# louisaslett/PhaseType

Hardware: NVIDIA B200
Metric: path_draws_per_sec (higher is better)
Workload: dtype f64

## Files before the change

### phasetype_b200/csrc/k_mhrs.cu

```cuda
#include <cooperative_groups.h>
#include "engine_internal.h"
#include "pht_philox.h"

namespace cg = cooperative_groups;

#ifndef MHRS_THREADS
#define MHRS_THREADS 256
#endif
#define MHRS_WARPS (MHRS_THREADS / 32)
#ifndef MHRS_MIN_BLOCKS
#define MHRS_MIN_BLOCKS 4
#endif
#ifndef MHRS_TAIL_MIN_BLOCKS
#define MHRS_TAIL_MIN_BLOCKS 3
#endif
#ifndef MHRS_NOINLINE_COLD
#define MHRS_COLD static __device__ __forceinline__
#else
#define MHRS_COLD static __device__ __noinline__
#endif
#define GUIDE_BITS 8
#define GUIDE (1 << GUIDE_BITS)
#ifndef END_CAP
#define END_CAP 32u
#endif
#ifndef MHRS_REPLAY_MIN_BLOCKS
#define MHRS_REPLAY_MIN_BLOCKS 4
#endif
#ifndef REPLAY_REFILL_MIN
#define REPLAY_REFILL_MIN 16
#endif
#ifndef EV_MIN
#define EV_MIN 8u
#endif
#ifndef EV_WAIT
#define EV_WAIT 16u
#endif
#ifndef PREFETCH_MIN
#define PREFETCH_MIN 8
#endif
#ifndef TAIL_CH
#define TAIL_CH 256u
#endif
#ifndef TAIL_BATCH
#define TAIL_BATCH 1u
#endif
#ifndef TAIL_LATE_P
#define TAIL_LATE_P 1024u
#endif
#ifndef TAIL_LATE_GROWTH
#define TAIL_LATE_GROWTH 4u
#endif
#ifndef DRAIN_LANES
#define DRAIN_LANES 32
#endif
#ifndef TAIL_K0
#define TAIL_K0 512u
#endif
#define TAIL_KMAX (1u << 24)
#ifndef TAIL_GROWTH
#define TAIL_GROWTH 2u
#endif
#ifndef FOUND_PERIOD
#define FOUND_PERIOD 8u
#endif
#define POOL_MIN 32u
#ifndef POOL_MAX
#define POOL_MAX 256u
#endif
#define FOUND_NONE 0xFFFFFFFFFFFFFFFFull
#define T52_NEVER (1ull << 52)
#define LOWBITS (1u << 20)
#define XBAR_TIMEOUT_NS 4000000000ull

#define RF_PROP 2u
#define RF_OFF 4u
#define RF_SKIP 8u

template <int NC>
struct MhrsSmem {
    static constexpr int R = NC + 1;
    unsigned long long thr[R * R];
    double cum[R * R];
    double scale[NC];
    double s[NC];
    double inv_smax;
    unsigned long long zlo[NC];
    long long zhi[NC];
    unsigned int Nacc[NC * NC];
    unsigned int Bacc[NC];
    float A[R + 3];
    unsigned int paths_done;
    unsigned int scan[MHRS_WARPS + 1];
    uint32_t pctr[MHRS_WARPS];
    float pf_yf[MHRS_THREADS]; uint32_t pf_og[MHRS_THREADS], pf_pos[MHRS_THREADS];
    uint32_t mh_cur_a[MHRS_THREADS], mh_misc[MHRS_THREADS];
    unsigned char guide[R * GUIDE];
};

__device__ __forceinline__ unsigned long long gtimer() {
    unsigned long long t; asm volatile("mov.u64 %0, %globaltimer;" : "=l"(t)); return t;
}
__device__ __forceinline__ float lg2_approx(float x) {
    float r; asm("lg2.approx.ftz.f32 %0, %1;" : "=f"(r) : "f"(x)); return r;
}

__device__ __forceinline__ pht_u32x4 philox_block(uint32_t c0, uint32_t c1, uint32_t c2, uint32_t c3, const SweepParams &p) {
    PHT_PHILOX_ROUND(p.rk.k[0], p.rk.k[1])   PHT_PHILOX_ROUND(p.rk.k[2], p.rk.k[3])   PHT_PHILOX_ROUND(p.rk.k[4], p.rk.k[5])
    PHT_PHILOX_ROUND(p.rk.k[6], p.rk.k[7])   PHT_PHILOX_ROUND(p.rk.k[8], p.rk.k[9])   PHT_PHILOX_ROUND(p.rk.k[10], p.rk.k[11])
    PHT_PHILOX_ROUND(p.rk.k[12], p.rk.k[13]) PHT_PHILOX_ROUND(p.rk.k[14], p.rk.k[15]) PHT_PHILOX_ROUND(p.rk.k[16], p.rk.k[17])
    PHT_PHILOX_ROUND(p.rk.k[18], p.rk.k[19])
    pht_u32x4 out; out.v[0] = c0; out.v[1] = c1; out.v[2] = c2; out.v[3] = c3;
    return out;
}

struct Walk {
    double t, spare;
    uint32_t spare_hi, a, b;
    int j;
    bool odd, fresh;
};
struct Rec { double lastt; int B; long out_idx; double *z2; };

__device__ __forceinline__ void walk_begin(Walk &w, uint32_t a, bool off, uint32_t og, const SweepParams &p, uint32_t iter) {
    w.a = a; w.fresh = true; w.b = 0; w.odd = false; w.t = 0.0; w.j = 0; w.spare = 0.0; w.spare_hi = 0u;
    if (off) {
        pht_u32x4 r = philox_block(0u, a, og, iter, p);
        w.spare = pht_u01(r.v[2], r.v[3]); w.spare_hi = r.v[3]; w.odd = true; w.b = 1;
    }
}

__device__ __forceinline__ double log_unit(double x) { return pht_log_core(pht_d2u(x), 0); }

template <bool RECORD, int NC>
__device__ __forceinline__ bool walk_step(Walk &w, double y, bool cens, uint32_t og, const SweepParams &p, MhrsSmem<NC> &sm,
                                          uint32_t iter, int n, Rec &rec) {
    constexpr int R = NC + 1;
    pht_u32x4 r = philox_block(w.b, w.a, og, iter, p);
    w.b++;
    const double f = pht_u01(r.v[0], r.v[1]), g = pht_u01(r.v[2], r.v[3]);
    const double uA = w.odd ? w.spare : f;
    const uint32_t hiA = w.odd ? w.spare_hi : r.v[1];
    const double uB = w.odd ? f : g;
    w.spare = g; w.spare_hi = r.v[3];
    const bool fresh = w.fresh;
    const int row = fresh ? n : w.j;
    const int last = fresh ? n - 1 : n;
    const double *c = sm.cum + row * R;
    int k = sm.guide[row * GUIDE + (hiA >> (32 - GUIDE_BITS))] & 0x7f;
    while (k < last && c[k] < uA) k++;
    const bool cont = (k < n) && (w.t < y || cens);
    const bool ended = !fresh && !cont;
    const bool advance = !fresh && cont;
    if (RECORD) {
        if (advance) {
            rec.z2[w.j] += w.t - rec.lastt;
            if (p.outN != nullptr) p.outN[(size_t)rec.out_idx * n * n + w.j + k * n]++;
            else atomicAdd(&sm.Nacc[w.j + k * n], 1u);
        }
        rec.lastt = fresh ? 0.0 : (advance ? w.t : rec.lastt);
        rec.B = fresh ? k : rec.B;
    }
    const double tb = fresh ? 0.0 : w.t;
    const int jn = ended ? w.j : k;
    const double tn = tb + sm.scale[jn] * (-log_unit(uB));
    w.t = ended ? w.t : tn;
    w.j = jn;
    w.fresh = false;
    return ended;
}

template <int NC, bool IV = false>
MHRS_COLD uint32_t exact_attempt(uint32_t a, bool off, double y, bool cens, uint32_t og, const SweepParams &p,
                                                      MhrsSmem<NC> &sm, uint32_t iter, int n, uint32_t smask, double u = 0.0) {
    Walk w; Rec norec; norec.lastt = 0.0; norec.B = 0; norec.out_idx = 0; norec.z2 = nullptr;
    walk_begin(w, a, off, og, p, iter);
    unsigned st = 1;
    while (!walk_step<false>(w, y, cens, og, p, sm, iter, n, norec)) st++;
    bool ok = (w.t >= y) && ((smask >> w.j) & 1u);
    if constexpr (IV) ok = ok && w.t <= u;
    return (ok ? 1u : 0u) | ((uint32_t)w.j << 8) | ((st > 0xffffu ? 0xffffu : st) << 16);
}

template <int NC>
__device__ __forceinline__ void replay_phase(const SweepParams &p, MhrsSmem<NC> &sm, uint32_t iter, int n,
                                             uint32_t obs_begin, uint32_t obs_end, unsigned &c_jumps) {
    const unsigned FULL = 0xffffffffu; const int lane = threadIdx.x & 31;
    constexpr bool LANE_Z = NC <= 8;
    long long ztot[LANE_Z ? NC : 1];
#pragma unroll
    for (int i = 0; i < (LANE_Z ? NC : 1); i++) ztot[i] = 0;
    double z2[NC];
    Walk w; Rec rec; rec.lastt = 0.0; rec.B = 0; rec.z2 = z2; rec.out_idx = 0;
    w.t = 0.0; w.spare = 0.0; w.spare_hi = 0u; w.a = 0u; w.b = 0u; w.j = 0; w.odd = false; w.fresh = true;
    double y = 0.0; bool cens = false, act = false, fin = false, dry = false, bad = false; uint32_t og = 0u;
    unsigned paths = 0;
    const double zs = pht_u2d((uint64_t)(1023 + p.zbits) << 52);
    for (;;) {
        const unsigned idle = __ballot_sync(FULL, !act);
        if (idle == FULL || (unsigned)__popc(idle) >= REPLAY_REFILL_MIN) {
            if (fin) {
                fin = false; paths++;
                z2[w.j] += (cens ? w.t : y) - rec.lastt;
                if (p.outB != nullptr) {
                    p.outB[rec.out_idx] = rec.B;
                    p.outN[rec.out_idx * n * n + w.j + w.j * n]++;
#pragma unroll 1
                    for (int i = 0; i < n; i++) p.outz[rec.out_idx * n + i] = z2[i];
                } else {
                    atomicAdd(&sm.Nacc[w.j + w.j * n], 1u); atomicAdd(&sm.Bacc[rec.B], 1u);
#pragma unroll
                    for (int i = 0; i < NC; i++) {
                        if (i < n) {
                            const double v = z2[i];
                            bad = bad || !(v * zs < 4.0e18);
                            const long long fx = __double2ll_rn(v * zs);
                            if (LANE_Z) { ztot[LANE_Z ? i : 0] += fx; bad = bad || ztot[LANE_Z ? i : 0] < 0; }
                            else if (fx != 0) pht_zfix_add(sm.zlo, sm.zhi, i, fx);
                        }
                    }
                }
            }
            if (!dry) {
                const unsigned cnt = __popc(idle);
                unsigned long long base = 0;
                if (lane == 0) base = (unsigned long long)obs_begin + atomicAdd(&p.state->replay_next, (unsigned long long)cnt);
                base = __shfl_sync(FULL, base, 0);
                const unsigned long long left = base < obs_end ? (unsigned long long)obs_end - base : 0ull;
                const unsigned avail = left < cnt ? (unsigned)left : cnt;
                if (avail < cnt) dry = true;
                const unsigned rank = __popc(idle & ((1u << lane) - 1u));
                if (!act && rank < avail) {
                    const unsigned long long pos = base + rank;
                    const uint4 r = p.recs[pos];
                    if (!(r.z & RF_SKIP)) {
                        const uint32_t obs_local = p.perm ? p.perm[pos] : (uint32_t)pos;
                        y = p.y[pos]; cens = p.cens[pos] != 0; og = p.obs_rank + obs_local * p.obs_world;
                        rec.out_idx = (long)obs_local - p.first; rec.lastt = 0.0; rec.B = 0;
                        uint32_t a = r.x;
                        if (r.z & RF_PROP) {
                            const pht_u32x4 q = philox_block(0u, r.y + 1u, og, iter, p);
                            const double U = pht_u01(q.v[0], q.v[1]);
                            if (U < sm.s[(r.z >> 16) & 0xffu] / sm.s[(r.z >> 8) & 0xffu]) a = r.y;
                        }
#pragma unroll
                        for (int i = 0; i < NC; i++) z2[i] = 0.0;
                        walk_begin(w, a, (r.z & RF_OFF) != 0u, og, p, iter);
                        act = true;
                    }
                }
            }
        }
        if (__ballot_sync(FULL, act) == 0u) { if (dry) break; else continue; }
        __syncwarp();
        if (act) { c_jumps++; if (walk_step<true>(w, y, cens, og, p, sm, iter, n, rec)) { act = false; fin = true; } }
    }
    if (p.outB == nullptr) {
        if (LANE_Z) {
#pragma unroll
            for (int i = 0; i < NC; i++) {
                if (i < n) {
                    const long long fx = ztot[LANE_Z ? i : 0];
                    unsigned long long lo = (unsigned long long)fx & 0xffffffffull; long long hi = fx >> 32;
                    for (int d = 16; d > 0; d >>= 1) { lo += __shfl_xor_sync(FULL, lo, d); hi += __shfl_xor_sync(FULL, hi, d); }
                    if (lane == 0 && (lo | (unsigned long long)hi)) {
                        atomicAdd(&sm.zlo[i], lo); atomicAdd(reinterpret_cast<unsigned long long *>(&sm.zhi[i]), (unsigned long long)hi);
                    }
                }
            }
        }
        if (bad) atomicOr(&p.state->error, 2);
    }
    for (int d = 16; d > 0; d >>= 1) paths += __shfl_xor_sync(FULL, paths, d);
    if (lane == 0 && paths) atomicAdd(&sm.paths_done, paths);
}

struct ObsF { float yn; uint32_t og; bool cens; };
__device__ __forceinline__ void obs_set(ObsF &o, float yn, uint32_t og, bool cens) { o.yn = yn; o.og = og; o.cens = cens; }
struct ObsFU : ObsF { float un, bn; };
template <bool IV> struct ObsOf { typedef ObsF T; };
template <> struct ObsOf<true> { typedef ObsFU T; };
__device__ __forceinline__ void obs_set_u(ObsF &, float) {}
__device__ __forceinline__ void obs_set_u(ObsFU &o, float un) { o.un = un; o.bn = (un < __int_as_float(0x7f800000)) ? un : o.yn; }
__device__ __forceinline__ float obs_bound(const ObsF &o) { return o.yn; }
__device__ __forceinline__ float obs_bound(const ObsFU &o) { return o.bn; }
template <bool IV> __device__ __forceinline__ double upper_at(const double *u, uint32_t pos) {
    if constexpr (IV) return u[pos]; else return 0.0;
}
struct Fast { float t, dacc; uint32_t a, b; int row; };

__device__ __forceinline__ void fast_begin(Fast &f, uint32_t a, int n) { f.t = 0.0f; f.dacc = 0.0f; f.a = a; f.b = 0u; f.row = n; }

template <int NC, bool IV = false>
__device__ __forceinline__ void fast_step(Fast &f, const typename ObsOf<IV>::T &o, const SweepParams &p, const MhrsSmem<NC> &sm, uint32_t iter, int n,
                                          bool &fail, bool &surv, bool &amb, int &kout) {
    constexpr int R = NC + 1;
    const pht_u32x4 r = philox_block(f.b, f.a, o.og, iter, p);
    f.b++;
    const unsigned long long x = (((unsigned long long)r.v[1] << 32) | r.v[0]) >> 12;
    const unsigned g = sm.guide[f.row * GUIDE + (r.v[1] >> (32 - GUIDE_BITS))];
    int k = (int)(g & 0x7fu);
    if (!(g & 0x80u)) { const unsigned long long *th = sm.thr + f.row * R; while (x >= th[k]) k++; }
    const uint32_t w = r.v[3];
    const uint32_t wb = __float_as_uint(__uint2float_rn(w));
    const uint32_t eb = wb >> 23;
    const float lg2m = lg2_approx(__uint_as_float((wb & 0x007fffffu) | 0x3f800000u));
    const float L = (__uint_as_float(0x4b400000u + eb) - 12583071.0f) + lg2m;
    f.t = __fmaf_rn(L, sm.A[k], f.t);
    const float trunc = __uint_as_float((254u - eb) << 23);
    const float c0y = __fmaf_rn(1.2e-7f, obs_bound(o), 4.5e-7f);
    const float step_err = __fmaf_rn(trunc, 2.0f, __fmaf_rn(fabsf(L), 2.5e-7f, c0y));
    const bool flagged = (w < 4096u) || (f.b >> 12) != 0u;
    f.dacc = flagged ? __int_as_float(0x7f800000) : f.dacc + step_err;
    const bool absd = (k == n);
    const float diff = f.t - o.yn;
    const bool over = diff > f.dacc, under = -diff > f.dacc;
    const bool test = o.cens == absd;
    surv = test && over;
    amb = test && !over && !under;
    fail = absd && (!o.cens || under);
    if constexpr (IV) {
        const float du = f.t - o.un;
        const bool past = du > f.dacc, below = -du > f.dacc;
        fail = fail || past;
        amb = test && !under && !past && !(over && below);
        surv = surv && below;
    }
    kout = absd ? f.row : k;
    f.row = k;
}

template <int NC>
__device__ __forceinline__ void build_tables(const SweepParams &p, MhrsSmem<NC> &sm, int n, const ModelLayout &ML) {
    constexpr int R = NC + 1;
    const int tid = threadIdx.x;
    double smax = 0.0;
    for (int i = 0; i < n; i++) { const double sc = p.model[ML.scale + i]; smax = (sc > smax) ? sc : smax; }
    const double inv_smax = 1.0 / smax;
    for (int i = tid; i < n; i += MHRS_THREADS) {
        const double sc = p.model[ML.scale + i];
        sm.scale[i] = sc; sm.s[i] = p.model[ML.s + i]; sm.zlo[i] = 0ull; sm.zhi[i] = 0; sm.Bacc[i] = 0u;
        sm.A[i] = (float)((-0.69314718055994530942 * sc) * inv_smax);
    }
    if (tid == 0) { sm.A[n] = 0.0f; sm.inv_smax = inv_smax; }
    for (int i = tid; i < n * n; i += MHRS_THREADS) sm.Nacc[i] = 0u;
    for (int e = tid; e < R * R; e += MHRS_THREADS) {
        const int row = e / R, k = e % R;
        unsigned long long t52 = T52_NEVER; double c = 0.0;
        if (row <= n && k <= n) {
            c = p.model[ML.cum + row * (n + 1) + k];
            const int last = (row == n) ? n - 1 : n;
            if (k < last && c < 1.0) {
                if (!(c > 0.0)) t52 = 0ull;
                else {
                    const unsigned long long xf = (unsigned long long)(c * 4503599627370496.0);
                    const double u = pht_u2d(0x3ff0000000000000ULL | xf) - 0.99999999999999988898;
                    t52 = (u > c) ? xf : xf + 1ull;
                }
            }
        }
        sm.thr[e] = t52; sm.cum[e] = c;
    }
    if (tid == 0) sm.paths_done = 0u;
    __syncthreads();
    for (int e = tid; e < (n + 1) * GUIDE; e += MHRS_THREADS) {
        const int row = e / GUIDE, b = e % GUIDE, last = (row == n) ? n - 1 : n;
        const double floor_u = (double)b * (1.0 / GUIDE);
        int k = 0;
        while (k < last && sm.cum[row * R + k] <= floor_u) k++;
        const bool pure = sm.thr[row * R + k] >= ((unsigned long long)(b + 1) << (52 - GUIDE_BITS));
        sm.guide[e] = (unsigned char)(k | (pure ? 0x80 : 0));
    }
    __syncthreads();
}

__device__ __forceinline__ uint32_t pack_flags(bool have_cur, bool cur_off, bool off, bool cens, int cur_pre, uint32_t kprop) {
    return (have_cur ? TI_HAVE : 0u) | (cur_off ? TI_CUROFF : 0u) | (off ? TI_OFF : 0u) | (cens ? TI_CENS : 0u) |
           ((uint32_t)(cur_pre & 0xff) << 8) | (kprop << 16);
}

__device__ __forceinline__ void peer_barrier(cg::grid_group &grid, const SweepParams &p, unsigned long long epoch) {
    const unsigned long long t_in = (blockIdx.x == 0 && threadIdx.x == 0) ? gtimer() : 0ull;
    __threadfence_system();
    grid.sync();
    if (blockIdx.x == 0) {
        const int t = threadIdx.x;
        if (t < (int)p.obs_world && p.state->xdead == 0u) {
            volatile unsigned long long *mine = &p.xpeer[t]->flags[p.obs_rank];
            __threadfence_system();
            *mine = epoch;
            __threadfence_system();
            volatile unsigned long long *theirs = &p.xw->flags[t];
            const unsigned long long t0 = gtimer();
            while (*theirs < epoch) {
                if (gtimer() - t0 > XBAR_TIMEOUT_NS) { p.state->xdead = 1u; atomicOr(&p.state->error, 64); break; }
            }
            __threadfence_system();
        }
    }
    grid.sync();
    if (blockIdx.x == 0 && threadIdx.x == 0) atomicAdd(&p.state->counters[PHT_CNT_NS_XWAIT], gtimer() - t_in);
}

struct TailView {
    TailItem *items; const uint32_t *pend; unsigned long long *found; uint32_t P, K;
    bool global; uint32_t parity;
    const double *u;
};

template <int NC, bool IV = false>
__device__ __forceinline__ void tail_search(const TailView &tv, const SweepParams &p, MhrsSmem<NC> &sm, uint32_t iter, int n,
                                            uint32_t smask, uint32_t nwarps,
                                            unsigned &c_jumps, unsigned &c_attempts) {
    const unsigned FULL = 0xffffffffu; const int lane = threadIdx.x & 31;
    const uint32_t W = tv.global ? p.obs_world : 1u;
    const uint32_t Pl = (tv.P + W - 1u) / W;
    const unsigned long long total_units = (unsigned long long)Pl * tv.K;
    Fast f; fast_begin(f, 0u, n);
    typename ObsOf<IV>::T mo; obs_set(mo, 0.0f, 0u, false); obs_set_u(mo, 0.0f);
    uint32_t my_item = 0xFFFFFFFFu; bool active = false;
    unsigned steps = 0;
    uint32_t *ctr = &sm.pctr[threadIdx.x >> 5];
    if (lane == 0) *ctr = 0u;
    __syncwarp();
    unsigned long long u_next = 0, u_end = 0, last_base = 0, remaining = total_units;
    bool out_of_units = false, finished = false;
    uint32_t item = 0, og = 0, a_first = 0, pool_end = 0; float yf = 0.0f, uf = 0.0f; bool cens = false, first_off = false;
    while (!finished) {
        bool want_exact = false, exact_off = false, survived = false; int kend = 0;
#define TAIL_GRAB() do { \
            const uint32_t na_ = atomicAdd(ctr, 1u); \
            if (na_ < pool_end) { \
                my_item = item; obs_set(mo, yf, og, cens); obs_set_u(mo, uf); fast_begin(f, na_, n); \
                 \
                if (first_off && na_ == a_first) { want_exact = true; exact_off = true; active = false; } else active = true; \
            } else active = false; \
        } while (0)
        for (;;) {
            const unsigned idle = __ballot_sync(FULL, !active);
            if (idle) {
                uint32_t cur = *reinterpret_cast<volatile uint32_t *>(ctr);
                if (cur >= pool_end && !out_of_units) {
                    bool have = false; uint32_t pstart = 0u;
                    while (!have) {
                        if (u_next >= u_end) {
                            remaining = total_units > last_base ? total_units - last_base : 0ull;
                            unsigned long long want = remaining / (2ull * (unsigned long long)nwarps);
                            want = want < POOL_MIN ? POOL_MIN : (want > POOL_MAX ? POOL_MAX : want);
                            unsigned long long base = 0;
                            if (lane == 0) base = atomicAdd(&p.state->unit_counter, want);
                            base = __shfl_sync(FULL, base, 0);
                            last_base = base;
                            if (base >= total_units) { out_of_units = true; break; }
                            u_next = base; u_end = base + want < total_units ? base + want : total_units;
                        }
                        const unsigned long long chunk = u_next / TAIL_CH;
                        const unsigned long long chunk_end_u = (chunk + 1ull) * TAIL_CH;
                        const unsigned long long stop = u_end < chunk_end_u ? u_end : chunk_end_u;
                        const uint32_t q = (uint32_t)(chunk / Pl), col = (uint32_t)(chunk % Pl);
                        const uint32_t o = tv.global ? col * W + (p.obs_rank + W - q % W) % W : col;
                        const uint32_t within = (uint32_t)(u_next - chunk * TAIL_CH), len = (uint32_t)(stop - u_next);
                        u_next = stop;
                        if (o >= tv.P) continue;
                        const uint32_t it_idx = tv.pend[o];
                        const TailItem it = tv.items[it_idx];
                        if (it.flags & TI_FIN) continue;
                        pstart = it.a + q * TAIL_CH + within;
                        if ((__ldcg(&tv.found[it_idx]) >> 8) >= (unsigned long long)pstart) {
                            have = true;
                            item = it_idx; a_first = it.a; first_off = (it.flags & TI_OFF) != 0u;
                            pool_end = pstart + len;
                            yf = (float)(it.y * sm.inv_smax); cens = (it.flags & TI_CENS) != 0u; og = it.og;
                            if constexpr (IV) uf = (float)(tv.u[it_idx] * sm.inv_smax);
                        }
                    }
                    if (have) {
                        __syncwarp();
                        if (lane == 0) *ctr = pstart;
                        __syncwarp();
                        cur = pstart;
                    }
                }
                if (cur >= pool_end) { if (idle == FULL) { finished = true; break; } }
                else if (!active) TAIL_GRAB();
            }
            if (((++steps) & (FOUND_PERIOD - 1u)) == 0u) {
                unsigned long long fw = 0;
                if (lane == 0) fw = __ldcg(&tv.found[item]);
                fw = __shfl_sync(FULL, fw, 0);
                if (fw != FOUND_NONE) {
                    const uint32_t fa = (uint32_t)(fw >> 8);
                    pool_end = pool_end < fa ? pool_end : fa;
                    if (my_item == item && active && f.a > fa) { active = false; c_jumps += f.b; }
                }
            }
            __syncwarp();
            if (active) {
                bool fail, surv, amb; int k;
                fast_step<NC, IV>(f, mo, p, sm, iter, n, fail, surv, amb, k);
                if (surv && !((smask >> k) & 1u)) { surv = false; fail = true; }
                if (fail) { c_attempts++; c_jumps += f.b; TAIL_GRAB(); }
                else if (surv) { c_attempts++; c_jumps += f.b; survived = true; kend = k; active = false; }
                else if (amb) { c_jumps += f.b; want_exact = true; active = false; }
            }
            if (__any_sync(FULL, survived || want_exact)) break;
        }
#undef TAIL_GRAB
        if (finished) break;
        if (want_exact) {
            const uint32_t res = exact_attempt<NC, IV>(f.a, exact_off, tv.items[my_item].y, mo.cens, mo.og, p, sm, iter, n, smask,
                                                       upper_at<IV>(tv.u, my_item));
            c_jumps += res >> 16; c_attempts++;
            survived = res & 1u; kend = (int)((res >> 8) & 0xffu);
        }
        const unsigned smk = __ballot_sync(FULL, survived);
        if (survived) {
            const unsigned long long word = ((unsigned long long)f.a << 8) | (unsigned long long)kend;
            atomicMin(&tv.found[my_item], word);
            if (tv.global) {
                for (uint32_t r = 0; r < p.obs_world; r++)
                    if (r != p.obs_rank) atomicMin_system(&p.xpeer[r]->gfound[tv.parity][my_item], word);
                __threadfence_system();
            }
        }
        if (smk) {
            const int src = __ffs(smk) - 1;
            const uint32_t s_item = __shfl_sync(FULL, my_item, src), s_a = __shfl_sync(FULL, f.a, src);
            if (my_item == s_item && active && f.a > s_a) { active = false; c_jumps += f.b; }
            if (s_item == item) pool_end = pool_end < s_a ? pool_end : s_a;
        }
        __syncwarp();
    }
}

MHRS_COLD int tail_advance(TailItem &it, unsigned long long fword, uint32_t K, const SweepParams &p,
                                            const double *s_model, uint32_t iter, bool &failed) {
    failed = false;
    if (fword == FOUND_NONE) {
        failed = true;
        if (it.a > 0xF0000000u - K) return 2;
        it.a += K; it.flags &= ~TI_OFF;
        return 0;
    }
    const uint32_t a = (uint32_t)(fword >> 8); const int pre = (int)(fword & 0xffull);
    const bool off = (a == it.a) && (it.flags & TI_OFF);
    const bool cens = (it.flags & TI_CENS) != 0u;
    bool have_cur = it.flags & TI_HAVE; bool cur_off = it.flags & TI_CUROFF;
    int cur_pre = (int)((it.flags >> 8) & 0xffu); uint32_t kprop = it.flags >> 16;
    bool next_off = false, done;
    if (!have_cur) {
        have_cur = true; it.cur_a = a; cur_off = off; cur_pre = pre;
        done = cens || p.mhit == 0;
    } else {
        pht_u32x4 r = philox_block(0u, a + 1u, it.og, iter, p);
        const double U = pht_u01(r.v[0], r.v[1]);
        if (U < s_model[pre] / s_model[cur_pre]) { it.cur_a = a; cur_off = off; cur_pre = pre; }
        kprop++; done = (int)kprop >= p.mhit; next_off = true;
    }
    it.a = a + 1u;
    it.flags = pack_flags(have_cur, cur_off, next_off, cens, cur_pre, kprop);
    return done ? 1 : 0;
}

#define LF_RUN 1u
#define LF_HAVE 2u
// ... 7 lines not shown
    const unsigned FULL = 0xffffffffu;
    const int tid = threadIdx.x, lane = tid & 31;
    Fast f; fast_begin(f, 0u, n);
    typename ObsOf<IV>::T o; obs_set(o, 0.0f, 0u, false); obs_set_u(o, 0.0f);
    const double inv_smax = sm.inv_smax;
    uint32_t pos = 0, a_lim = cap, fl = 0u;
    bool dry = false;
    for (;;) {
        const unsigned empty = __ballot_sync(FULL, !(fl & LF_NVALID));
        if (!dry && __popc(empty) >= PREFETCH_MIN) {
            const unsigned cnt = __popc(empty);
            unsigned long long base = 0;
            if (lane == 0) base = (unsigned long long)obs_begin + atomicAdd(&p.state->next_obs, (unsigned long long)cnt);
            base = __shfl_sync(FULL, base, 0);
            const unsigned long long left = base < obs_end ? (unsigned long long)obs_end - base : 0ull;
            const unsigned avail = left < cnt ? (unsigned)left : cnt;
            if (avail < cnt) dry = true;
            const unsigned rank = __popc(empty & ((1u << lane) - 1u));
            if (!(fl & LF_NVALID) && rank < avail) {
                const unsigned long long q = base + rank;
                sm.pf_pos[tid] = (uint32_t)q; sm.pf_yf[tid] = (float)(p.y[q] * inv_smax);
                sm.pf_og[tid] = p.obs_rank + (p.perm ? p.perm[q] : (uint32_t)q) * p.obs_world;
                fl |= LF_NVALID | (p.cens[q] != 0 ? LF_NCENS : 0u);
            }
        }
        if (!(fl & LF_RUN) && (fl & LF_NVALID)) {
            obs_set(o, sm.pf_yf[tid], sm.pf_og[tid], (fl & LF_NCENS) != 0u); pos = sm.pf_pos[tid];
            if constexpr (IV) obs_set_u(o, (float)(p.u[pos] * inv_smax));
            fl = LF_RUN | (o.cens ? LF_CENS : 0u);
            sm.mh_cur_a[tid] = 0u; sm.mh_misc[tid] = 0u; a_lim = cap;
            fast_begin(f, 0u, n);
        }
        const unsigned running = __ballot_sync(FULL, fl & LF_RUN);
        if (running == 0u) { if (dry) break; else continue; }
        if (dry && __popc(running) <= DRAIN_LANES && a_lim != 0xFFFFFFFFu && a_lim > END_CAP) a_lim = END_CAP;
        __syncwarp();
        bool surv = false, amb = false, hand = false; int k = 0;
        bool go = (fl & LF_RUN) != 0u;
        unsigned waited = 0u, ev;
        do {
            if (go) {
                bool fail;
                fast_step<NC, IV>(f, o, p, sm, iter, n, fail, surv, amb, k);
                if (fail) { c_jumps += f.b; fast_begin(f, f.a + 1u, n); c_attempts++; hand = f.a >= a_lim; }
                go = !(surv || amb || hand);
            }
            ev = __ballot_sync(FULL, !go);
            waited += ((ev & running) != 0u) ? 1u : 0u;
        } while (ev != 0xffffffffu && (unsigned)__popc(ev & running) < EV_MIN && waited < EV_WAIT);
        if (surv || amb) c_jumps += f.b;
        if (amb) {
            const uint32_t res = exact_attempt<NC, IV>(f.a, false, p.y[pos], o.cens, o.og, p, sm, iter, n, ~0u, upper_at<IV>(p.u, pos));
            surv = res & 1u; k = (int)((res >> 8) & 0xffu); c_jumps += res >> 16;
            if (!surv) { fast_begin(f, f.a + 1u, n); c_attempts++; hand = f.a >= a_lim; }
        }
        if (surv && !((smask >> k) & 1u)) { surv = false; fast_begin(f, f.a + 1u, n); c_attempts++; hand = f.a >= a_lim; }
        bool this_off = false;
        while (surv) {
            c_attempts++;
            bool complete = false; uint32_t rfl = 0u, ra1 = 0u, ra2 = 0u;
            uint32_t cur_a = sm.mh_cur_a[tid], misc = sm.mh_misc[tid];
            int cur_pre = (int)(misc & 0xffu); bool cur_off = (misc >> 8) & 1u; uint32_t kprop = misc >> 16;
            if (!(fl & LF_HAVE)) {
                fl |= LF_HAVE; cur_a = f.a; cur_off = this_off; cur_pre = k;
                if (o.cens || p.mhit == 0) { complete = true; ra1 = cur_a; rfl = cur_off ? RF_OFF : 0u; }
            } else if (p.mhit == 1) {
                complete = true; ra1 = cur_a; ra2 = f.a;
                rfl = RF_PROP | ((uint32_t)cur_pre << 8) | ((uint32_t)k << 16);
            } else {
                pht_u32x4 r = philox_block(0u, f.a + 1u, o.og, iter, p);
                const double U = pht_u01(r.v[0], r.v[1]);
                if (U < sm.s[k] / sm.s[cur_pre]) { cur_a = f.a; cur_off = this_off; cur_pre = k; }
                kprop++;
                if ((int)kprop >= p.mhit) { complete = true; ra1 = cur_a; rfl = cur_off ? RF_OFF : 0u; }
            }
            sm.mh_cur_a[tid] = cur_a; sm.mh_misc[tid] = (uint32_t)cur_pre | (cur_off ? 0x100u : 0u) | (kprop << 16);
            if (complete) {
                p.recs[pos] = make_uint4(ra1, ra2, rfl, 0u);
                fl &= ~LF_RUN; surv = false;
            } else if (kprop == 0u) {
                fast_begin(f, f.a + 1u, n); surv = false;
            } else {
                const uint32_t a = f.a + 1u;
                const uint32_t res = exact_attempt<NC, IV>(a, true, p.y[pos], o.cens, o.og, p, sm, iter, n, smask, upper_at<IV>(p.u, pos));
                surv = res & 1u; k = (int)((res >> 8) & 0xffu); c_jumps += res >> 16;
                this_off = true;
                if (!surv) c_attempts++;
                fast_begin(f, surv ? a : a + 1u, n);
            }
        }
        if (hand && (fl & LF_RUN)) {
            const uint32_t idx = atomicAdd(&p.state->n_items, 1u);
            if (idx < p.item_cap) {
                const uint32_t misc = sm.mh_misc[tid];
                TailItem it; it.y = p.y[pos]; it.og = o.og; it.pos = pos; it.a = f.a; it.cur_a = sm.mh_cur_a[tid];
                it.flags = pack_flags((fl & LF_HAVE) != 0u, (misc >> 8) & 1u, false, o.cens, (int)(misc & 0xffu), misc >> 16);
                it.owner = p.obs_rank;
                p.items[idx] = it; p.found[idx] = FOUND_NONE;
                if constexpr (IV) p.item_u[idx] = p.u[pos];
                atomicAdd(&p.state->counters[PHT_CNT_DEFERRED], 1ull);
                fl &= ~LF_RUN;
            } else a_lim = 0xFFFFFFFFu;
        }
        __syncwarp();
    }
}

template <int NC>
__device__ __forceinline__ void flush_block(const SweepParams &p, MhrsSmem<NC> &sm, int n, bool stats, unsigned c_attempts, unsigned c_jumps) {
    const unsigned FULL = 0xffffffffu; const int tid = threadIdx.x;
    __syncthreads();
    if (stats) {
        unsigned long long *gN = reinterpret_cast<unsigned long long *>(p.stats);
        for (int i = tid; i < n * n; i += MHRS_THREADS) if (sm.Nacc[i]) atomicAdd(&gN[i], (unsigned long long)sm.Nacc[i]);
        for (int i = tid; i < n; i += MHRS_THREADS) {
            if (sm.Bacc[i]) atomicAdd(&gN[n * n + i], (unsigned long long)sm.Bacc[i]);
            if (sm.zlo[i]) atomicAdd(&gN[n * n + n + i], sm.zlo[i]);
            if (sm.zhi[i]) atomicAdd(&gN[n * n + 2 * n + i], (unsigned long long)sm.zhi[i]);
        }
    }
    unsigned long long w_attempts = c_attempts, w_jumps = c_jumps;
    for (int o = 16; o > 0; o >>= 1) { w_attempts += __shfl_down_sync(FULL, w_attempts, o); w_jumps += __shfl_down_sync(FULL, w_jumps, o); }
    if ((tid & 31) == 0) { atomicAdd(&p.state->counters[PHT_CNT_ATTEMPTS], w_attempts); atomicAdd(&p.state->counters[PHT_CNT_JUMPS], w_jumps); }
    if (tid == 0 && sm.paths_done) atomicAdd(&p.state->counters[PHT_CNT_PATHS], (unsigned long long)sm.paths_done);
}

template <int NC>
__device__ __forceinline__ void model_scalars(const MhrsSmem<NC> &sm, int n, uint32_t &smask) {
    smask = 0u;
    for (int i = 0; i < n; i++) smask |= (sm.s[i] != 0.0) ? (1u << i) : 0u;
}

template <int NC, bool IV>
__global__ void __launch_bounds__(MHRS_THREADS, MHRS_MIN_BLOCKS) k_mhrs_lanes(const __grid_constant__ SweepParams p) {
    extern __shared__ __align__(16) unsigned char smem_raw[];
    MhrsSmem<NC> &sm = *reinterpret_cast<MhrsSmem<NC> *>(smem_raw);
    const int n = p.n;
    const uint32_t iter = p.state->iter;
    const unsigned long long t0 = (blockIdx.x == 0 && threadIdx.x == 0) ? gtimer() : 0ull;
    build_tables(p, sm, n, ModelLayout::make(n, p.m));
    uint32_t smask;
    model_scalars(sm, n, smask);
    const bool per_obs = p.outB != nullptr;
    const uint32_t obs_begin = per_obs ? (uint32_t)p.first : 0u;
    const uint32_t obs_end = per_obs ? (uint32_t)(p.first + p.count) : (uint32_t)p.l_local;
    const uint32_t cap = p.mhrs_cap > 0 ? (uint32_t)p.mhrs_cap : 256u;
    unsigned c_attempts = 0, c_jumps = 0;
    lane_phase<NC, IV>(p, sm, iter, n, smask, obs_begin, obs_end, cap, c_jumps, c_attempts);
    flush_block(p, sm, n, false, c_attempts, c_jumps);
    if (blockIdx.x == 0 && threadIdx.x == 0) atomicAdd(&p.state->counters[PHT_CNT_NS_LANE], gtimer() - t0);
}

template <int NC, bool IV>
__global__ void __launch_bounds__(MHRS_THREADS, MHRS_TAIL_MIN_BLOCKS) k_mhrs_tail(const __grid_constant__ SweepParams p) {
    extern __shared__ __align__(16) unsigned char smem_raw[];
    cg::grid_group grid = cg::this_grid();
    MhrsSmem<NC> &sm = *reinterpret_cast<MhrsSmem<NC> *>(smem_raw);
    const int n = p.n, tid = threadIdx.x;
    const uint32_t iter = p.state->iter;
    const bool per_obs = p.outB != nullptr;
    const bool multi = p.xw != nullptr && p.obs_world > 1u && !per_obs;
    const uint32_t n_items = p.state->n_items < p.item_cap ? p.state->n_items : p.item_cap;
    if (n_items == 0u && !multi) return;
    const bool timekeeper = (blockIdx.x == 0 && tid == 0);
    unsigned long long t_mark = timekeeper ? gtimer() : 0ull;
    build_tables(p, sm, n, ModelLayout::make(n, p.m));
    uint32_t smask;
    model_scalars(sm, n, smask);
    const double *s_model = p.model + ModelLayout::make(n, p.m).s;
    unsigned c_attempts = 0, c_jumps = 0;
    const uint32_t gtid = blockIdx.x * MHRS_THREADS + tid, gsize = gridDim.x * MHRS_THREADS, nwarps = gsize / 32u;

    for (uint32_t i = gtid; i < n_items; i += gsize) p.pend0[i] = i;
    if (gtid == 0) {
        p.state->n_pend[0] = n_items; p.state->n_pend[1] = 0u; p.state->unit_counter = 0ull;
        p.state->any_fail[0] = 0u; p.state->any_fail[1] = 0u;
    }
    grid.sync();
    uint32_t K = TAIL_K0; while (K < (uint32_t)p.mhrs_cap && K < TAIL_KMAX) K *= 2u;
    uint32_t rounds = 0u, g0 = 0u, Pg = 0u; int cur = 0, gl_cur = 0; bool global = false;
    const uint32_t W = p.obs_world, me = p.obs_rank, sp = iter & 1u;
    unsigned long long epoch = multi ? p.state->xepoch : 0ull;
    for (;;) {
        const uint32_t *pend = cur ? p.pend1 : p.pend0;
        uint32_t *pend_next = cur ? p.pend0 : p.pend1;
        if (!global) {
            const uint32_t P = p.state->n_pend[cur];
            const bool leave = P == 0u || (multi && K >= p.k_switch && P <= PHT_GCAP);
            if (leave && !multi) break;
            if (leave) {
                if (timekeeper) { const unsigned long long t = gtimer(); atomicAdd(&p.state->counters[PHT_CNT_NS_TAIL], t - t_mark); t_mark = t; }
                for (uint32_t r = 0; r < W; r++) {
                    XchgWindow *dst = p.xpeer[r];
                    for (uint32_t i = gtid; i < P; i += gsize) {
                        dst->gitems[sp][me * PHT_GCAP + i] = p.items[pend[i]];
                        if constexpr (IV) dst->gitem_u[sp][me * PHT_GCAP + i] = p.item_u[pend[i]];
                    }
                    if (gtid == 0) dst->gcount[sp][me] = P;
                }
                peer_barrier(grid, p, ++epoch);
                for (uint32_t r = 0; r < W; r++) {
                    const uint32_t c = p.xw->gcount[sp][r] <= PHT_GCAP ? p.xw->gcount[sp][r] : PHT_GCAP;
                    for (uint32_t i = gtid; i < c; i += gsize) p.glist[Pg + i] = r * PHT_GCAP + i;
                    Pg += c;
                }
                if (gtid == 0) {
                    p.state->n_gpend = Pg; p.state->unit_counter = 0ull; p.state->any_fail[0] = 0u; p.state->any_fail[1] = 0u;
                    atomicAdd(&p.state->counters[PHT_CNT_GLOBAL_ITEMS], (unsigned long long)Pg);
                }
                grid.sync();
                global = true; g0 = rounds;
                K = p.k_switch > TAIL_K0 ? p.k_switch : TAIL_K0;
                continue;
            }
        } else if (Pg == 0u || p.state->xdead != 0u) break;
        const uint32_t par = (rounds - g0) & 1u;
        TailView tv;
        if (!global) { tv.items = p.items; tv.pend = pend; tv.found = p.found; tv.P = p.state->n_pend[cur]; tv.u = p.item_u; }
        else { tv.items = p.xw->gitems[sp]; tv.pend = gl_cur ? p.glist + PHT_MAX_WORLD * PHT_GCAP : p.glist; tv.found = p.xw->gfound[par]; tv.P = Pg; tv.u = p.xw->gitem_u[sp]; }
        tv.K = K; tv.global = global; tv.parity = par;
        const unsigned long long tr0 = timekeeper ? gtimer() : 0ull;
        const unsigned att0 = c_attempts, jmp0 = c_jumps;
        tail_search<NC, IV>(tv, p, sm, iter, n, smask, nwarps, c_jumps, c_attempts);
        const unsigned long long tr1 = timekeeper ? gtimer() : 0ull;
        if (rounds < PHT_ROUND_TRACE) {
            unsigned d = c_attempts - att0;
            for (int o = 16; o > 0; o >>= 1) d += __shfl_xor_sync(0xffffffffu, d, o);
            if ((tid & 31) == 0 && d) atomicAdd(&p.state->round_trace[rounds][5], (unsigned long long)d);
            unsigned dj = c_jumps - jmp0;
            for (int o = 16; o > 0; o >>= 1) dj += __shfl_xor_sync(0xffffffffu, dj, o);
            if ((tid & 31) == 0 && dj) atomicAdd(&p.state->round_trace[rounds][7], (unsigned long long)dj);
        }
        if (global) peer_barrier(grid, p, ++epoch); else grid.sync();
        const unsigned long long tr2 = timekeeper ? gtimer() : 0ull;
        for (uint32_t i = gtid; i < tv.P; i += gsize) {
            const uint32_t item = tv.pend[i];
            TailItem it = tv.items[item];
            if (it.flags & TI_FIN) continue;
            bool failed;
            if (rounds < PHT_ROUND_TRACE && (!global || it.owner == me)) {
                const unsigned long long fw = tv.found[item];
                atomicAdd(&p.state->round_trace[rounds][6], fw == FOUND_NONE ? (unsigned long long)K : (unsigned long long)((uint32_t)(fw >> 8) - it.a + 1u));
            }
            const int st = tail_advance(it, tv.found[item], K, p, s_model, iter, failed);
            tv.found[item] = FOUND_NONE;
            if (st != 0 && global) it.flags |= TI_FIN;
            tv.items[item] = it;
            const bool mine = !global || it.owner == me;
            if (st == 2 && mine) { atomicAdd(&p.state->counters[PHT_CNT_ERRORS], 1ull); atomicOr(&p.state->error, 8); }
            if (failed && st == 0) atomicOr(&p.state->any_fail[par], 1u);
            if (st != 0 && mine) p.recs[it.pos] = (st == 1) ? make_uint4(it.cur_a, 0u, (it.flags & TI_CUROFF) ? RF_OFF : 0u, 0u) : make_uint4(0u, 0u, RF_SKIP, 0u);
            if (st == 0 && !global) pend_next[atomicAdd(&p.state->n_pend[cur ^ 1], 1u)] = item;
        }
        if (gtid == 0) { if (!global) p.state->n_pend[cur] = 0u; p.state->unit_counter = 0ull; p.state->any_fail[par ^ 1u] = 0u; }
        grid.sync();
        if (global) {
            uint32_t *next_list = (gl_cur ? p.glist : p.glist + PHT_MAX_WORLD * PHT_GCAP);
            if (blockIdx.x == 0) {
                const int lane = tid & 31, warp = tid >> 5;
                uint32_t outn = 0u;
                for (uint32_t tile = 0; tile < Pg; tile += MHRS_THREADS) {
                    const uint32_t i = tile + tid;
                    uint32_t item = 0u; bool keep = false;
                    if (i < Pg) { item = tv.pend[i]; keep = !(tv.items[item].flags & TI_FIN); }
                    const unsigned bal = __ballot_sync(0xffffffffu, keep);
                    if (lane == 0) sm.scan[warp] = __popc(bal);
                    __syncthreads();
                    uint32_t off = 0u, tot = 0u;
                    for (int w2 = 0; w2 < MHRS_WARPS; w2++) { const uint32_t c = sm.scan[w2]; off += (w2 < warp) ? c : 0u; tot += c; }
                    if (keep) next_list[outn + off + __popc(bal & ((1u << lane) - 1u))] = item;
                    outn += tot;
                    __syncthreads();
                }
                if (tid == 0) p.state->n_gpend = outn;
            }
            grid.sync();
            Pg = p.state->n_gpend; gl_cur ^= 1;
        }
        const bool grow = p.state->any_fail[par] != 0u;
        if (timekeeper && rounds < PHT_ROUND_TRACE) {
            unsigned long long *tr = p.state->round_trace[rounds];
            tr[0] += tr1 - tr0; tr[1] += tr2 - tr1; tr[2] += gtimer() - tr2; tr[3] += tv.P; tr[4] += K;
        }
        if (!global) cur ^= 1;
        rounds++;
        if (grow && K < TAIL_KMAX) K *= ((global ? Pg : p.state->n_pend[cur]) <= TAIL_LATE_P) ? TAIL_LATE_GROWTH : TAIL_GROWTH;
        if (K > TAIL_KMAX) K = TAIL_KMAX;
    }
    if (multi && gtid == 0) { p.state->xepoch = epoch; p.state->n_pend[cur] = 0u; }
    if (timekeeper) {
        const unsigned long long t = gtimer();
        atomicAdd(&p.state->counters[global ? PHT_CNT_NS_GLOBAL : PHT_CNT_NS_TAIL], t - t_mark); t_mark = t;
    }
    if (gtid == 0) {
        atomicAdd(&p.state->counters[PHT_CNT_TAIL_ROUNDS], (unsigned long long)rounds);
        if (global) atomicAdd(&p.state->counters[PHT_CNT_GLOBAL_ROUNDS], (unsigned long long)(rounds - g0));
    }
    flush_block(p, sm, n, false, c_attempts, c_jumps);
}

template <int NC>
__global__ void __launch_bounds__(MHRS_THREADS, MHRS_REPLAY_MIN_BLOCKS) k_mhrs_replay(const __grid_constant__ SweepParams p) {
    extern __shared__ __align__(16) unsigned char smem_raw[];
    MhrsSmem<NC> &sm = *reinterpret_cast<MhrsSmem<NC> *>(smem_raw);
    const int n = p.n;
    const uint32_t iter = p.state->iter;
    const unsigned long long t0 = (blockIdx.x == 0 && threadIdx.x == 0) ? gtimer() : 0ull;
    build_tables(p, sm, n, ModelLayout::make(n, p.m));
    const bool per_obs = p.outB != nullptr;
    const uint32_t obs_begin = per_obs ? (uint32_t)p.first : 0u;
    const uint32_t obs_end = per_obs ? (uint32_t)(p.first + p.count) : (uint32_t)p.l_local;
    unsigned c_jumps = 0;
    replay_phase(p, sm, iter, n, obs_begin, obs_end, c_jumps);
    flush_block(p, sm, n, !per_obs, 0u, c_jumps);
    if (blockIdx.x == 0 && threadIdx.x == 0) atomicAdd(&p.state->counters[PHT_CNT_NS_REPLAY], gtimer() - t0);
}

template <int NC, bool IV>
static int grid_blocks_of(int device, int *lane_blocks, int *tail_blocks, int *replay_blocks) {
    int a = 0, b = 0, c = 0, sms = 0;
    const size_t smem = sizeof(MhrsSmem<NC>);
    if (cudaFuncSetAttribute(k_mhrs_lanes<NC, IV>, cudaFuncAttributeMaxDynamicSharedMemorySize, (int)smem) != cudaSuccess) return -1;
    if (cudaFuncSetAttribute(k_mhrs_tail<NC, IV>, cudaFuncAttributeMaxDynamicSharedMemorySize, (int)smem) != cudaSuccess) return -1;
    if (cudaOccupancyMaxActiveBlocksPerMultiprocessor(&a, k_mhrs_lanes<NC, IV>, MHRS_THREADS, smem) != cudaSuccess) return -1;
    if (cudaOccupancyMaxActiveBlocksPerMultiprocessor(&b, k_mhrs_tail<NC, IV>, MHRS_THREADS, smem) != cudaSuccess) return -1;
    if (cudaFuncSetAttribute(k_mhrs_replay<NC>, cudaFuncAttributeMaxDynamicSharedMemorySize, (int)smem) != cudaSuccess) return -1;
    if (cudaOccupancyMaxActiveBlocksPerMultiprocessor(&c, k_mhrs_replay<NC>, MHRS_THREADS, smem) != cudaSuccess) return -1;
    if (cudaDeviceGetAttribute(&sms, cudaDevAttrMultiProcessorCount, device) != cudaSuccess) return -1;
    *lane_blocks = a * sms; *tail_blocks = b * sms; *replay_blocks = c * sms;
    return (a > 0 && b > 0 && c > 0) ? 0 : -1;
}
int pht_mhrs_grid_blocks(int device, int n, bool iv, int *lane_blocks, int *tail_blocks, int *replay_blocks) {
    if (iv) {
        if (n <= 8) return grid_blocks_of<8, true>(device, lane_blocks, tail_blocks, replay_blocks);
        if (n <= 16) return grid_blocks_of<16, true>(device, lane_blocks, tail_blocks, replay_blocks);
        return grid_blocks_of<32, true>(device, lane_blocks, tail_blocks, replay_blocks);
    }
    if (n <= 8) return grid_blocks_of<8, false>(device, lane_blocks, tail_blocks, replay_blocks);
    if (n <= 16) return grid_blocks_of<16, false>(device, lane_blocks, tail_blocks, replay_blocks);
    return grid_blocks_of<32, false>(device, lane_blocks, tail_blocks, replay_blocks);
}
size_t pht_mhrs_smem_bytes(int n) {
    return n <= 8 ? sizeof(MhrsSmem<8>) : (n <= 16 ? sizeof(MhrsSmem<16>) : sizeof(MhrsSmem<32>));
}

template <int NC, bool IV>
static cudaError_t launch_of(const SweepParams &p, int lane_blocks, int tail_blocks, int replay_blocks, cudaStream_t st) {
    SweepParams q = p;
    void *args[] = { &q };
    const size_t smem = sizeof(MhrsSmem<NC>);
    k_mhrs_lanes<NC, IV><<<lane_blocks, MHRS_THREADS, smem, st>>>(q);
    cudaError_t e = cudaGetLastError();
    if (e != cudaSuccess) return e;
    e = cudaLaunchCooperativeKernel((const void *)k_mhrs_tail<NC, IV>, dim3(tail_blocks), dim3(MHRS_THREADS), args, smem, st);
    if (e != cudaSuccess) return e;
    k_mhrs_replay<NC><<<replay_blocks, MHRS_THREADS, smem, st>>>(q);
    return cudaGetLastError();
}
cudaError_t pht_launch_mhrs(const SweepParams &p, int lane_blocks, int tail_blocks, int replay_blocks, cudaStream_t st) {
    if (p.u != nullptr) {
        if (p.n <= 8) return launch_of<8, true>(p, lane_blocks, tail_blocks, replay_blocks, st);
        if (p.n <= 16) return launch_of<16, true>(p, lane_blocks, tail_blocks, replay_blocks, st);
        return launch_of<32, true>(p, lane_blocks, tail_blocks, replay_blocks, st);
    }
    if (p.n <= 8) return launch_of<8, false>(p, lane_blocks, tail_blocks, replay_blocks, st);
    if (p.n <= 16) return launch_of<16, false>(p, lane_blocks, tail_blocks, replay_blocks, st);
    return launch_of<32, false>(p, lane_blocks, tail_blocks, replay_blocks, st);
}
```

Measured before the change: 881.1 million.

## Prefetch replay records via cp.async and move per-thread path state to shared memory

Replay workers now prefetch their next observation record, y and perm entry into shared-memory slots with cp.async while the current walk runs, which hides global load latency at refill time. Per-path z accumulators and fixed-point totals move from registers or local memory into shared-memory slabs, reducing register pressure and local spills. The categorical search uses 52-bit integer thresholds with a guide-table exact-hit flag instead of double comparisons. Replay shared memory grows, which may reduce occupancy, and the integer threshold table (sm.thr) must match what build_tables produces.

```diff
diff --git a/phasetype_b200/csrc/k_mhrs.cu b/phasetype_b200/csrc/k_mhrs.cu
--- a/phasetype_b200/csrc/k_mhrs.cu
+++ b/phasetype_b200/csrc/k_mhrs.cu
@@ -120,7 +120,6 @@
     int j;
     bool odd, fresh;
 };
-struct Rec { double lastt; int B; long out_idx; double *z2; };
 
 __device__ __forceinline__ void walk_begin(Walk &w, uint32_t a, bool off, uint32_t og, const SweepParams &p, uint32_t iter) {
     w.a = a; w.fresh = true; w.b = 0; w.odd = false; w.t = 0.0; w.j = 0; w.spare = 0.0; w.spare_hi = 0u;
@@ -132,9 +131,9 @@
 
 __device__ __forceinline__ double log_unit(double x) { return pht_log_core(pht_d2u(x), 0); }
 
-template <bool RECORD, int NC>
+template <int NC>
 __device__ __forceinline__ bool walk_step(Walk &w, double y, bool cens, uint32_t og, const SweepParams &p, MhrsSmem<NC> &sm,
-                                          uint32_t iter, int n, Rec &rec) {
+                                          uint32_t iter, int n) {
     constexpr int R = NC + 1;
     pht_u32x4 r = philox_block(w.b, w.a, og, iter, p);
     w.b++;
@@ -151,16 +150,6 @@
     while (k < last && c[k] < uA) k++;
     const bool cont = (k < n) && (w.t < y || cens);
     const bool ended = !fresh && !cont;
-    const bool advance = !fresh && cont;
-    if (RECORD) {
-        if (advance) {
-            rec.z2[w.j] += w.t - rec.lastt;
-            if (p.outN != nullptr) p.outN[(size_t)rec.out_idx * n * n + w.j + k * n]++;
-            else atomicAdd(&sm.Nacc[w.j + k * n], 1u);
-        }
-        rec.lastt = fresh ? 0.0 : (advance ? w.t : rec.lastt);
-        rec.B = fresh ? k : rec.B;
-    }
     const double tb = fresh ? 0.0 : w.t;
     const int jn = ended ? w.j : k;
     const double tn = tb + sm.scale[jn] * (-log_unit(uB));
@@ -173,27 +162,107 @@
 template <int NC, bool IV = false>
 MHRS_COLD uint32_t exact_attempt(uint32_t a, bool off, double y, bool cens, uint32_t og, const SweepParams &p,
                                                       MhrsSmem<NC> &sm, uint32_t iter, int n, uint32_t smask, double u = 0.0) {
-    Walk w; Rec norec; norec.lastt = 0.0; norec.B = 0; norec.out_idx = 0; norec.z2 = nullptr;
+    Walk w;
     walk_begin(w, a, off, og, p, iter);
     unsigned st = 1;
-    while (!walk_step<false>(w, y, cens, og, p, sm, iter, n, norec)) st++;
+    while (!walk_step(w, y, cens, og, p, sm, iter, n)) st++;
     bool ok = (w.t >= y) && ((smask >> w.j) & 1u);
     if constexpr (IV) ok = ok && w.t <= u;
     return (ok ? 1u : 0u) | ((uint32_t)w.j << 8) | ((st > 0xffffu ? 0xffffu : st) << 16);
 }
 
+struct RWalk {
+    double t;
+    unsigned long long spare;
+    uint32_t a, b;
+    int j;
+    bool odd, fresh;
+};
+struct Rec { double lastt; int B; long out_idx; };
+
+__device__ __forceinline__ unsigned long long bits52(uint32_t lo, uint32_t hi) { return (((unsigned long long)hi << 32) | lo) >> 12; }
+
+__device__ __forceinline__ void rwalk_begin(RWalk &w, uint32_t a, bool off, uint32_t og, const SweepParams &p, uint32_t iter) {
+    w.a = a; w.fresh = true; w.b = 0; w.odd = false; w.t = 0.0; w.j = 0; w.spare = 0ull;
+    if (off) {
+        const pht_u32x4 r = philox_block(0u, a, og, iter, p);
+        w.spare = bits52(r.v[2], r.v[3]); w.odd = true; w.b = 1;
+    }
+}
+
+template <int NC, int ZS>
+__device__ __forceinline__ bool replay_step(RWalk &w, double y, bool cens, uint32_t og, const SweepParams &p, const MhrsSmem<NC> &sm,
+                                            uint32_t iter, int n, Rec &rec, double *z2, unsigned *Nacc) {
+    constexpr int R = NC + 1;
+    const pht_u32x4 r = philox_block(w.b, w.a, og, iter, p);
+    w.b++;
+    const unsigned long long xA = w.odd ? w.spare : bits52(r.v[0], r.v[1]);
+    const double uB = w.odd ? pht_u01(r.v[0], r.v[1]) : pht_u01(r.v[2], r.v[3]);
+    w.spare = bits52(r.v[2], r.v[3]);
+    const bool fresh = w.fresh;
+    const int row = fresh ? n : w.j;
+    const unsigned g = sm.guide[row * GUIDE + (unsigned)(xA >> (52 - GUIDE_BITS))];
+    int k = (int)(g & 0x7fu);
+    if (!(g & 0x80u)) { const unsigned long long *th = sm.thr + row * R; while (xA >= th[k]) k++; }
+    const bool cont = (k < n) && (w.t < y || cens);
+    const bool ended = !fresh && !cont;
+    const bool advance = !fresh && cont;
+    if (advance) {
+        z2[w.j * ZS] += w.t - rec.lastt;
+        if (p.outN != nullptr) p.outN[(size_t)rec.out_idx * n * n + w.j + k * n]++;
+        else atomicAdd(&Nacc[w.j + k * n], 1u);
+    }
+    rec.lastt = fresh ? 0.0 : (advance ? w.t : rec.lastt);
+    rec.B = fresh ? k : rec.B;
+    const double tb = fresh ? 0.0 : w.t;
+    const int jn = ended ? w.j : k;
+    const double tn = tb + sm.scale[jn] * (-log_unit(uB));
+    w.t = ended ? w.t : tn;
+    w.j = jn;
+    w.fresh = false;
+    return ended;
+}
+
+#ifndef REPLAY_Z_SLAB_MAX
+#define REPLAY_Z_SLAB_MAX 16
+#endif
 template <int NC>
-__device__ __forceinline__ void replay_phase(const SweepParams &p, MhrsSmem<NC> &sm, uint32_t iter, int n,
+struct ReplaySmem {
+    static constexpr bool Z_SLAB = NC <= REPLAY_Z_SLAB_MAX;
+    MhrsSmem<NC> t;
+    uint4 pf_rec[MHRS_THREADS];
+    double pf_y[MHRS_THREADS];
+    uint32_t pf_obs[MHRS_THREADS];
+    double z2[Z_SLAB ? NC : 1][Z_SLAB ? MHRS_THREADS : 1];
+    long long zfx[NC <= 8 ? NC : 1][NC <= 8 ? MHRS_THREADS : 1];
+};
+
+__device__ __forceinline__ void cp_async16(void *dst, const void *src) {
+    asm volatile("cp.async.cg.shared.global [%0], [%1], 16;" :: "r"((uint32_t)__cvta_generic_to_shared(dst)), "l"(src) : "memory");
+}
+__device__ __forceinline__ void cp_async8(void *dst, const void *src) {
+    asm volatile("cp.async.ca.shared.global [%0], [%1], 8;" :: "r"((uint32_t)__cvta_generic_to_shared(dst)), "l"(src) : "memory");
+}
+__device__ __forceinline__ void cp_async4(void *dst, const void *src) {
+    asm volatile("cp.async.ca.shared.global [%0], [%1], 4;" :: "r"((uint32_t)__cvta_generic_to_shared(dst)), "l"(src) : "memory");
+}
+__device__ __forceinline__ void cp_async_wait() { asm volatile("cp.async.wait_all;" ::: "memory"); }
+
+template <int NC>
+__device__ __forceinline__ void replay_phase(const SweepParams &p, ReplaySmem<NC> &rs, uint32_t iter, int n,
                                              uint32_t obs_begin, uint32_t obs_end, unsigned &c_jumps) {
-    const unsigned FULL = 0xffffffffu; const int lane = threadIdx.x & 31;
+    MhrsSmem<NC> &sm = rs.t;
+    const unsigned FULL = 0xffffffffu; const int tid = threadIdx.x, lane = tid & 31;
     constexpr bool LANE_Z = NC <= 8;
-    long long ztot[LANE_Z ? NC : 1];
+    constexpr int ZS = ReplaySmem<NC>::Z_SLAB ? MHRS_THREADS : 1;
 #pragma unroll
-    for (int i = 0; i < (LANE_Z ? NC : 1); i++) ztot[i] = 0;
-    double z2[NC];
-    Walk w; Rec rec; rec.lastt = 0.0; rec.B = 0; rec.z2 = z2; rec.out_idx = 0;
-    w.t = 0.0; w.spare = 0.0; w.spare_hi = 0u; w.a = 0u; w.b = 0u; w.j = 0; w.odd = false; w.fresh = true;
+    for (int i = 0; i < (LANE_Z ? NC : 0); i++) rs.zfx[i][tid] = 0;
+    double z2_local[ReplaySmem<NC>::Z_SLAB ? 1 : NC];
+    double *z2 = ReplaySmem<NC>::Z_SLAB ? &rs.z2[0][tid] : z2_local;
+    RWalk w; Rec rec; rec.lastt = 0.0; rec.B = 0; rec.out_idx = 0;
+    w.t = 0.0; w.spare = 0ull; w.a = 0u; w.b = 0u; w.j = 0; w.odd = false; w.fresh = true;
     double y = 0.0; bool cens = false, act = false, fin = false, dry = false, bad = false; uint32_t og = 0u;
+    bool slot = false; uint32_t slot_cens = 0u;
     unsigned paths = 0;
     const double zs = pht_u2d((uint64_t)(1023 + p.zbits) << 52);
     for (;;) {
@@ -201,66 +270,77 @@
         if (idle == FULL || (unsigned)__popc(idle) >= REPLAY_REFILL_MIN) {
             if (fin) {
                 fin = false; paths++;
-                z2[w.j] += (cens ? w.t : y) - rec.lastt;
+                z2[w.j * ZS] += (cens ? w.t : y) - rec.lastt;
                 if (p.outB != nullptr) {
                     p.outB[rec.out_idx] = rec.B;
                     p.outN[rec.out_idx * n * n + w.j + w.j * n]++;
 #pragma unroll 1
-                    for (int i = 0; i < n; i++) p.outz[rec.out_idx * n + i] = z2[i];
+                    for (int i = 0; i < n; i++) p.outz[rec.out_idx * n + i] = z2[i * ZS];
                 } else {
                     atomicAdd(&sm.Nacc[w.j + w.j * n], 1u); atomicAdd(&sm.Bacc[rec.B], 1u);
 #pragma unroll
                     for (int i = 0; i < NC; i++) {
                         if (i < n) {
-                            const double v = z2[i];
+                            const double v = z2[i * ZS];
                             bad = bad || !(v * zs < 4.0e18);
                             const long long fx = __double2ll_rn(v * zs);
-                            if (LANE_Z) { ztot[LANE_Z ? i : 0] += fx; bad = bad || ztot[LANE_Z ? i : 0] < 0; }
+                            if constexpr (LANE_Z) { const long long zt = rs.zfx[i][tid] + fx; rs.zfx[i][tid] = zt; bad = bad || zt < 0; }
                             else if (fx != 0) pht_zfix_add(sm.zlo, sm.zhi, i, fx);
                         }
                     }
                 }
             }
-            if (!dry) {
-                const unsigned cnt = __popc(idle);
+            if (!act && slot) {
+                slot = false;
+                cp_async_wait();
+                const uint4 r = rs.pf_rec[tid];
+                if (!(r.z & RF_SKIP)) {
+                    const uint32_t obs_local = rs.pf_obs[tid];
+                    y = rs.pf_y[tid]; cens = slot_cens != 0u; og = p.obs_rank + obs_local * p.obs_world;
+                    rec.out_idx = (long)obs_local - p.first; rec.lastt = 0.0; rec.B = 0;
+                    uint32_t a = r.x;
+                    if (r.z & RF_PROP) {
+                        const pht_u32x4 q = philox_block(0u, r.y + 1u, og, iter, p);
+                        const double U = pht_u01(q.v[0], q.v[1]);
+                        if (U < sm.s[(r.z >> 16) & 0xffu] / sm.s[(r.z >> 8) & 0xffu]) a = r.y;
+                    }
+#pragma unroll
+                    for (int i = 0; i < NC; i++) z2[i * ZS] = 0.0;
+                    rwalk_begin(w, a, (r.z & RF_OFF) != 0u, og, p, iter);
+                    act = true;
+                }
+            }
+            const unsigned empty = __ballot_sync(FULL, !slot);
+            if (!dry && empty) {
+                const unsigned cnt = __popc(empty);
                 unsigned long long base = 0;
                 if (lane == 0) base = (unsigned long long)obs_begin + atomicAdd(&p.state->replay_next, (unsigned long long)cnt);
                 base = __shfl_sync(FULL, base, 0);
                 const unsigned long long left = base < obs_end ? (unsigned long long)obs_end - base : 0ull;
                 const unsigned avail = left < cnt ? (unsigned)left : cnt;
                 if (avail < cnt) dry = true;
-                const unsigned rank = __popc(idle & ((1u << lane) - 1u));
-                if (!act && rank < avail) {
+                const unsigned rank = __popc(empty & ((1u << lane) - 1u));
+                if (!slot && rank < avail) {
                     const unsigned long long pos = base + rank;
-                    const uint4 r = p.recs[pos];
-                    if (!(r.z & RF_SKIP)) {
-                        const uint32_t obs_local = p.perm ? p.perm[pos] : (uint32_t)pos;
-                        y = p.y[pos]; cens = p.cens[pos] != 0; og = p.obs_rank + obs_local * p.obs_world;
-                        rec.out_idx = (long)obs_local - p.first; rec.lastt = 0.0; rec.B = 0;
-                        uint32_t a = r.x;
-                        if (r.z & RF_PROP) {
-                            const pht_u32x4 q = philox_block(0u, r.y + 1u, og, iter, p);
-                            const double U = pht_u01(q.v[0], q.v[1]);
-                            if (U < sm.s[(r.z >> 16) & 0xffu] / sm.s[(r.z >> 8) & 0xffu]) a = r.y;
-                        }
-#pragma unroll
-                        for (int i = 0; i < NC; i++) z2[i] = 0.0;
-                        walk_begin(w, a, (r.z & RF_OFF) != 0u, og, p, iter);
-                        act = true;
-                    }
+                    cp_async16(&rs.pf_rec[tid], &p.recs[pos]);
+                    cp_async8(&rs.pf_y[tid], &p.y[pos]);
+                    if (p.perm) cp_async4(&rs.pf_obs[tid], &p.perm[pos]);
+                    else rs.pf_obs[tid] = (uint32_t)pos;
+                    slot_cens = p.cens[pos];
+                    slot = true;
                 }
             }
         }
-        if (__ballot_sync(FULL, act) == 0u) { if (dry) break; else continue; }
+        if (__ballot_sync(FULL, act) == 0u) { if (dry && __ballot_sync(FULL, slot) == 0u) break; else continue; }
         __syncwarp();
-        if (act) { c_jumps++; if (walk_step<true>(w, y, cens, og, p, sm, iter, n, rec)) { act = false; fin = true; } }
+        if (act) { c_jumps++; if (replay_step<NC, ZS>(w, y, cens, og, p, sm, iter, n, rec, z2, sm.Nacc)) { act = false; fin = true; } }
     }
     if (p.outB == nullptr) {
-        if (LANE_Z) {
+        if constexpr (LANE_Z) {
 #pragma unroll
             for (int i = 0; i < NC; i++) {
                 if (i < n) {
-                    const long long fx = ztot[LANE_Z ? i : 0];
+                    const long long fx = rs.zfx[i][tid];
                     unsigned long long lo = (unsigned long long)fx & 0xffffffffull; long long hi = fx >> 32;
                     for (int d = 16; d > 0; d >>= 1) { lo += __shfl_xor_sync(FULL, lo, d); hi += __shfl_xor_sync(FULL, hi, d); }
                     if (lane == 0 && (lo | (unsigned long long)hi)) {
@@ -874,17 +954,17 @@
 template <int NC>
 __global__ void __launch_bounds__(MHRS_THREADS, MHRS_REPLAY_MIN_BLOCKS) k_mhrs_replay(const __grid_constant__ SweepParams p) {
     extern __shared__ __align__(16) unsigned char smem_raw[];
-    MhrsSmem<NC> &sm = *reinterpret_cast<MhrsSmem<NC> *>(smem_raw);
+    ReplaySmem<NC> &rs = *reinterpret_cast<ReplaySmem<NC> *>(smem_raw);
     const int n = p.n;
     const uint32_t iter = p.state->iter;
     const unsigned long long t0 = (blockIdx.x == 0 && threadIdx.x == 0) ? gtimer() : 0ull;
-    build_tables(p, sm, n, ModelLayout::make(n, p.m));
+    build_tables(p, rs.t, n, ModelLayout::make(n, p.m));
     const bool per_obs = p.outB != nullptr;
     const uint32_t obs_begin = per_obs ? (uint32_t)p.first : 0u;
     const uint32_t obs_end = per_obs ? (uint32_t)(p.first + p.count) : (uint32_t)p.l_local;
     unsigned c_jumps = 0;
-    replay_phase(p, sm, iter, n, obs_begin, obs_end, c_jumps);
-    flush_block(p, sm, n, !per_obs, 0u, c_jumps);
+    replay_phase(p, rs, iter, n, obs_begin, obs_end, c_jumps);
+    flush_block(p, rs.t, n, !per_obs, 0u, c_jumps);
     if (blockIdx.x == 0 && threadIdx.x == 0) atomicAdd(&p.state->counters[PHT_CNT_NS_REPLAY], gtimer() - t0);
 }
 
@@ -896,8 +976,9 @@
     if (cudaFuncSetAttribute(k_mhrs_tail<NC, IV>, cudaFuncAttributeMaxDynamicSharedMemorySize, (int)smem) != cudaSuccess) return -1;
     if (cudaOccupancyMaxActiveBlocksPerMultiprocessor(&a, k_mhrs_lanes<NC, IV>, MHRS_THREADS, smem) != cudaSuccess) return -1;
     if (cudaOccupancyMaxActiveBlocksPerMultiprocessor(&b, k_mhrs_tail<NC, IV>, MHRS_THREADS, smem) != cudaSuccess) return -1;
-    if (cudaFuncSetAttribute(k_mhrs_replay<NC>, cudaFuncAttributeMaxDynamicSharedMemorySize, (int)smem) != cudaSuccess) return -1;
-    if (cudaOccupancyMaxActiveBlocksPerMultiprocessor(&c, k_mhrs_replay<NC>, MHRS_THREADS, smem) != cudaSuccess) return -1;
+    const size_t rsmem = sizeof(ReplaySmem<NC>);
+    if (cudaFuncSetAttribute(k_mhrs_replay<NC>, cudaFuncAttributeMaxDynamicSharedMemorySize, (int)rsmem) != cudaSuccess) return -1;
+    if (cudaOccupancyMaxActiveBlocksPerMultiprocessor(&c, k_mhrs_replay<NC>, MHRS_THREADS, rsmem) != cudaSuccess) return -1;
     if (cudaDeviceGetAttribute(&sms, cudaDevAttrMultiProcessorCount, device) != cudaSuccess) return -1;
     *lane_blocks = a * sms; *tail_blocks = b * sms; *replay_blocks = c * sms;
     return (a > 0 && b > 0 && c > 0) ? 0 : -1;
@@ -926,7 +1007,7 @@
     if (e != cudaSuccess) return e;
     e = cudaLaunchCooperativeKernel((const void *)k_mhrs_tail<NC, IV>, dim3(tail_blocks), dim3(MHRS_THREADS), args, smem, st);
     if (e != cudaSuccess) return e;
-    k_mhrs_replay<NC><<<replay_blocks, MHRS_THREADS, smem, st>>>(q);
+    k_mhrs_replay<NC><<<replay_blocks, MHRS_THREADS, sizeof(ReplaySmem<NC>), st>>>(q);
     return cudaGetLastError();
 }
 cudaError_t pht_launch_mhrs(const SweepParams &p, int lane_blocks, int tail_blocks, int replay_blocks, cudaStream_t st) {
```

Result: no change. 886.1 million (median of 6 runs) (+0.6%).
